# jltsiren/gcsa2

Measured on AMD Instinct MI355X. Metric: kmer_find_queries_per_sec, higher is better.
Workload: dtype u64; 1 GPU; whole-human-pangenome-sized index: order-17 de Bruijn graph of a degree-34 LFSR cycle of 5726623061 positions + junction edges between existing nodes (80 per mille of the candidates): 5726623061 path nodes, 6184749492 edges = 1.080 n; one batch of 100000000 x 32-mer find() sharded over 1 GPU(s), pattern set S (walks through the graph); edges=6184749492, queries_total=100000000, queries_per_gpu=100000000, pattern_len=32, index_bytes_hbm=209905278128, pair_block_bytes=61083979776, single_block_bytes=13362120576, kmer_table_k=16, block_bytes=128, pattern_set=S

## Files before the change

gcsa2_amd/csrc/gcsa2_hip.hip:

```cpp
#include "layout.hpp"
#include "sdsl_reader.hpp"
#include "sdsl_writer.hpp"
#include "../../include/gcsa2_hip.h"

#include <hipcub/hipcub.hpp>
#include <chrono>
#include <condition_variable>
#include <cstdio>
#include <cstdlib>
#include <cstring>
#include <algorithm>
#include <functional>
#include <atomic>
#include <memory>
#include <mutex>
#include <new>
#include <random>
#include <string>
#include <thread>
#include <unordered_set>
#include <vector>

using namespace g2;

// ... 2 lines not shown
#include "kernels_extend.hpp"
#include "kernels_locate.hpp"
#include "kernels_locate_max.hpp"
#include "kernels_mem.hpp"
#include "kernels_windows.hpp"
#include "kernels_lcp.hpp"
#include "kernels_submem.hpp"
#include "kernels_seeds.hpp"
#include "kernels_support.hpp"
#include "kernels_classes.hpp"
#include "kernels_mailbox.hpp"
#include "kernels_build.hpp"


constexpr unsigned RESULT_SLOTS = 1024;

struct Staging
{
  hipStream_t stream = nullptr;
  char* d = nullptr; size_t d_cap = 0;
  char* h = nullptr; size_t h_cap = 0;
  char* z = nullptr;
};

struct gcsa2_index
{
  int device = 0;
  DevImage img;
  void* d_base = nullptr;
  void* d_kmer = nullptr;
  void* d_pred4 = nullptr;
  void* d_locate = nullptr;
  void* d_jump = nullptr;
  void* d_pairs = nullptr;
  hipMemPool_t pool = nullptr;
  unsigned long long* d_slots = nullptr;
  unsigned long long* h_slots = nullptr;
  mutable std::atomic<unsigned> next_slot{0};
  mutable std::atomic<unsigned long long> next_ticket{1};
  mutable std::atomic<int> single_backoff{0};
  struct Mailbox { MailSlot* slot = nullptr; hipStream_t stream = nullptr; std::mutex lock; unsigned long long ticket = 0, launches = 0, calls = 0; bool failed = false; };
  mutable Mailbox mail;
  mutable std::mutex staging_lock;
  mutable std::vector<Staging*> staging_pool;
  int compute_units = 256;
  u64 bytes = 0;
  u64 order = 0;
  struct PipeSet { char* h = nullptr; char* d = nullptr; hipEvent_t done = nullptr; bool busy = false; u64 first = 0, count = 0; };
  struct PipeLane { hipStream_t stream = nullptr; PipeSet set[2]; };
  mutable std::mutex pipe_lock;
  mutable std::vector<PipeLane> pipe;
  struct Arena { char* base = nullptr; size_t bytes = 0; };
  mutable std::mutex arena_lock;
  mutable std::vector<Arena> arenas;
  struct Tuning
  {
    u32 cool_down = COOL_DOWN;
    u32 ms_refill_at = MS_REFILL_AT;
    u64 ms_grid = 0;
    u64 locate_split = (u64(1) << 31) - 1;
    u64 locate_split_queries = u64(1) << 30;
    u64 pipe_chunk = u64(1) << 18;
    u32 pipe_lanes = 6;
    u32 ms_threads = 4;
    u64 kmer_piece = u64(1) << 27;
    u64 ms_piece_bytes = u64(32) << 20;
    bool pipe_blocking = false;
    bool ms_pieces = true;
    bool zero_copy = true;
    u32 seed_wide = (u32(1) << 24) - 1;
    bool locate_trace = false;
    u32 split_target = SPLIT_TARGET;
    u32 split_skew = BIG_SEGMENT;
    bool locate_fused_compact = true;
    bool locate_single = true;
    bool locate_fuse = true;
    u64 fuse_above = BIG_SEGMENT;
    bool mailbox = true;
    u64 mailbox_park_us = 200;
    u64 mailbox_life_ms = 20;
    bool locate_in_place = true;
    size_t arena_cap = size_t(24) << 30;
    u64 budget_bytes = 0;
  } tune;
};

struct gcsa2_locate_job
{
  int device = 0;
  u64 nq = 0, total = 0;
  u64* d_offsets = nullptr;
  u64* d_values = nullptr;
  hipStream_t stream = nullptr;
};

namespace {

thread_local std::string g_error;

int fail(int code, const std::string& msg) { g_error = msg; return code; }

#define HIP_TRY(expr) do { hipError_t e_ = (expr); if(e_ != hipSuccess) { \
  return fail(e_ == hipErrorOutOfMemory ? GCSA2_ERR_OUT_OF_MEMORY : GCSA2_ERR_HIP, \
              std::string(#expr) + ": " + hipGetErrorString(e_)); } } while(0)

inline unsigned grid_for(u64 n) { return unsigned((n + TPB - 1) / TPB); }

inline u64 budget_left(const gcsa2_index* ix) { return ix->tune.budget_bytes > ix->bytes ? ix->tune.budget_bytes - ix->bytes : 0; }

constexpr bool JUMP_DEFAULT_FIND_ONLY = true;
inline bool jump_table_fits(u64 bytes, u64 free_bytes, u64 total_bytes) { return bytes <= free_bytes && free_bytes - bytes >= total_bytes / 16; }

inline void launch_walk(const gcsa2_index* ix, const u64* d_ranges, u64 nq, const u64* node_off, const u64* raw_off,
                        u64 total_nodes, u64* values, u64* owners, hipStream_t stream);


inline u64 pair_block_bytes_of(const DevImage& img) { return 16 * (img.n / PAIR_BITS + 1) * FLB_BYTES; }
inline bool pair_blocks_possible(const DevImage& img) { return img.sigma >= 5 && img.n > 0 && 16 * (img.n / PAIR_BITS + 1) < u64(PAIR_FLAG); }
inline bool seed_table_possible(const DevImage& img) { return img.sigma >= 5 && (img.n > img.e ? img.n : img.e) + 2 < (u64(1) << SEED_SP_BITS); }
inline bool locate_table_possible(const DevImage& img) { return img.has_samples && img.pred4 != nullptr && img.n > 0; }

void drop_pair_blocks(gcsa2_index* ix)
{
  if(ix->d_pairs != nullptr) { (void)hipFree(ix->d_pairs); ix->d_pairs = nullptr; ix->bytes -= pair_block_bytes_of(ix->img); }
  ix->img.flp = nullptr; ix->img.flp_nblocks = 0;
}

hipError_t make_pair_blocks(gcsa2_index* ix)
{
  drop_pair_blocks(ix);
  DevImage& img = ix->img;
  const u64 nb = img.n / PAIR_BITS + 1, pair_bytes = pair_block_bytes_of(img);
  hipError_t e = hipMalloc(&ix->d_pairs, pair_bytes);
  if(e == hipSuccess)
  {
    img.flp_nblocks = nb;
    const u64 slice = u64(1) << 20;
    for(u64 first = 0; first < nb && e == hipSuccess; first += slice)
    {
      const u64 count = (nb - first < slice ? nb - first : slice);
      hipLaunchKernelGGL(k_build_pair_blocks, dim3(unsigned(count), 4), dim3(unsigned(PAIR_BITS)), 0, nullptr, img, first, static_cast<u64*>(ix->d_pairs));
      e = hipGetLastError();
    }
    if(e == hipSuccess) { e = hipDeviceSynchronize(); }
  }
  if(e != hipSuccess)
  {
    if(ix->d_pairs != nullptr) { (void)hipFree(ix->d_pairs); ix->d_pairs = nullptr; }
    img.flp_nblocks = 0; (void)hipGetLastError();
    return e;
  }
  img.flp = static_cast<const u64*>(ix->d_pairs);
  ix->bytes += pair_bytes;
  return hipSuccess;
}

void drop_seed_table(gcsa2_index* ix)
{
  if(ix->d_kmer != nullptr) { (void)hipFree(ix->d_kmer); ix->d_kmer = nullptr; ix->bytes -= u64(8) << (2 * ix->img.kmer_k); }
  ix->img.kmer_table = nullptr; ix->img.kmer_k = 0;
}

hipError_t make_seed_table(gcsa2_index* ix, u32 k)
{
  drop_seed_table(ix);
  DevImage& img = ix->img;
// ... 475 lines not shown
  {
    if(v->char2comp[b] >= v->sigma) { return fail(GCSA2_ERR_INVALID_ARGUMENT, "alpha.char2comp maps a byte to a comp >= sigma"); }
  }
  for(u64 c = 0; c < v->sigma; c++)
  {
    if(v->C[c] > v->C[c + 1]) { return fail(GCSA2_ERR_INVALID_ARGUMENT, "alpha.C is not non-decreasing"); }
  }
  if(v->C[v->sigma] != v->edges) { return fail(GCSA2_ERR_INVALID_ARGUMENT, "alpha.C[sigma] differs from header.edges"); }
  if(v->sampled_path_bits != nullptr)
  {
    if(v->stored_samples == nullptr || v->sample_bits == nullptr || v->sample_width == 0 || v->sample_width > 64)
    {
      return fail(GCSA2_ERR_INVALID_ARGUMENT, "samples: missing array or sample width out of range");
    }
  }
  if(v->extra_filter_bits != nullptr && (v->extra_values_bits == nullptr || v->redundant_bits == nullptr))
  {
    return fail(GCSA2_ERR_INVALID_ARGUMENT, "counters: missing array");
  }
  if(v->lcp_data != nullptr)
  {
    if(v->lcp_offsets == nullptr || v->lcp_levels == 0) { return fail(GCSA2_ERR_INVALID_ARGUMENT, "LCP: missing offsets"); }
    if(v->lcp_branching < 2) { return fail(GCSA2_ERR_INVALID_ARGUMENT, "LCP: branching factor below 2"); }
    if(v->path_nodes > 0 && v->lcp_size != v->path_nodes) { return fail(GCSA2_ERR_INVALID_ARGUMENT, "LCP: header.size differs from the number of path nodes (an .lcp file of another index?)"); }
    u64 level_size = v->lcp_size, at = 0, top_size = 0;
    for(u64 l = 0; l < v->lcp_levels; l++)
    {
      if(v->lcp_offsets[l] != at) { return fail(GCSA2_ERR_INVALID_ARGUMENT, "LCP: offsets do not match the level sizes implied by the branching factor"); }
      at += level_size; top_size = level_size;
      if(l + 1 < v->lcp_levels && level_size <= 1) { return fail(GCSA2_ERR_INVALID_ARGUMENT, "LCP: levels above the root"); }
      level_size = (level_size + v->lcp_branching - 1) / v->lcp_branching;
    }
    if(v->lcp_offsets[v->lcp_levels] != at) { return fail(GCSA2_ERR_INVALID_ARGUMENT, "LCP: offsets do not match the level sizes implied by the branching factor"); }
    if(top_size > 1) { return fail(GCSA2_ERR_INVALID_ARGUMENT, "LCP: the top level is not a single root"); }
  }
  int count = gcsa2_device_count();
  if(count <= 0) { return fail(GCSA2_ERR_NO_DEVICE, "no HIP device visible: " + g_error); }
  if(device < 0 || device >= count) { return fail(GCSA2_ERR_INVALID_ARGUMENT, "device index out of range"); }

  if(v->sigma * (v->path_nodes / FLB_BITS + 1) >= u64(PAIR_FLAG) || v->lcp_size / 16 + 16 >= u64(PAIR_FLAG))
  {
    return fail(GCSA2_ERR_INVALID_ARGUMENT, "index too large: the block and LCP-window indices of the fetch keep two flag bits");
  }
  if(v->path_nodes > MAX_PATH_NODES || v->edges > 2 * MAX_PATH_NODES)
  {
    return fail(GCSA2_ERR_INVALID_ARGUMENT, "index of more than 2^38 path nodes: beyond what one device holds and what the block indices of this build address");
  }
  gcsa2_index* ix = new(std::nothrow) gcsa2_index();
  if(ix == nullptr) { return fail(GCSA2_ERR_OUT_OF_MEMORY, "host allocation failed"); }
  ix->device = device; ix->order = v->order;
  {
    auto knob = [](const char* name, long fallback, long lo, long hi) -> long
    {
      const char* e = std::getenv(name);
      long val = (e != nullptr && *e != 0 ? std::atol(e) : fallback);
      return val < lo ? lo : (val > hi ? hi : val);
    };
    ix->tune.cool_down = u32(knob("GCSA2_COOL_DOWN", COOL_DOWN, 0, 1000));
    ix->tune.ms_refill_at = u32(knob("GCSA2_MS_REFILL_AT", MS_REFILL_AT, 1, 64));
    ix->tune.ms_grid = u64(knob("GCSA2_MS_GRID", 0, 0, long(1) << 30));
    ix->tune.locate_split = u64(knob("GCSA2_LOCATE_SPLIT", (long(1) << 31) - 1, 2, (long(1) << 31) - 1));
    ix->tune.locate_split_queries = u64(knob("GCSA2_LOCATE_SPLIT_QUERIES", long(1) << 30, 1, long(1) << 30));
    ix->tune.zero_copy = (knob("GCSA2_ZERO_COPY", 1, 0, 1) != 0);
    ix->tune.pipe_lanes = u32(knob("GCSA2_PIPE_LANES", 6, 1, 16));
    ix->tune.pipe_chunk = u64(1) << knob("GCSA2_PIPE_CHUNK", 18, 15, 20);
    ix->tune.pipe_blocking = (knob("GCSA2_PIPE_BLOCKING", 0, 0, 1) != 0);
    ix->tune.ms_pieces = (knob("GCSA2_MS_PIECES", 1, 0, 1) != 0);
    ix->tune.ms_piece_bytes = u64(knob("GCSA2_MS_PIECE_MB", 32, 1, 1024)) << 20;
    ix->tune.ms_threads = u32(knob("GCSA2_MS_THREADS", 4, 1, 16));
    ix->tune.kmer_piece = u64(knob("GCSA2_KMER_PIECE", long(1) << 27, 4, long(1) << 27));
    ix->tune.locate_trace = (knob("GCSA2_LOCATE_TRACE", 0, 0, 1) != 0);
    ix->tune.locate_single = (knob("GCSA2_LOCATE_SINGLE", 1, 0, 1) != 0);
    ix->tune.locate_fused_compact = (knob("GCSA2_LOCATE_FUSED_COMPACT", 1, 0, 1) != 0);
    ix->tune.locate_fuse = (knob("GCSA2_LOCATE_FUSE", 1, 0, 1) != 0);
    ix->tune.fuse_above = u64(knob("GCSA2_LOCATE_FUSE_ABOVE", BIG_SEGMENT, 1, long(1) << 40));
    ix->tune.locate_in_place = (knob("GCSA2_LOCATE_IN_PLACE", 1, 0, 1) != 0);
    ix->tune.mailbox = (knob("GCSA2_MAILBOX", 1, 0, 1) != 0);
    ix->tune.mailbox_park_us = u64(knob("GCSA2_MAILBOX_PARK_US", 200, 1, 1000000));
    ix->tune.mailbox_life_ms = u64(knob("GCSA2_MAILBOX_LIFE_MS", 20, 1, 10000));
    ix->tune.split_skew = u32(knob("GCSA2_SPLIT_SKEW", BIG_SEGMENT, 16, BIG_SEGMENT));
    ix->tune.split_target = u32(knob("GCSA2_SPLIT_TARGET", SPLIT_TARGET, 1, 4096));
    ix->tune.arena_cap = size_t(knob("GCSA2_ARENA_CAP_MB", 24576, 0, long(1) << 20)) << 20;
    ix->tune.seed_wide = u32(knob("GCSA2_SEED_WIDE", long(SEED_WIDE), 2, long(SEED_WIDE)));
    {
      const char* b = std::getenv("GCSA2_MEMORY_BUDGET_MB");
      const double mb = (b != nullptr && *b != 0 ? std::atof(b) : 0.0);
      ix->tune.budget_bytes = (mb > 0.0 ? u64(mb * 1048576.0) : 0);
    }
  }
  std::memset(&ix->img, 0, sizeof(DevImage));
  DevImage& img = ix->img;
  img.n = v->path_nodes; img.e = v->edges; img.sigma = v->sigma; img.fast_chars = v->fast_chars;
  for(u64 c = 0; c <= v->sigma; c++) { img.C[c] = v->C[c]; }
  std::memcpy(img.char2comp, v->char2comp, 256);

  try
  {
    Planner pl;
    std::vector<BVPlan> bwt(v->sigma);
    for(u64 c = 0; c < v->sigma; c++)
    {
      bwt[c] = plan_bv(pl, img.n, false);
      if(c > 0 && bwt[c].blocks_off != bwt[0].blocks_off + c * (bwt[0].nblocks * BLOCK_WORDS))
      {
        delete ix; return fail(GCSA2_ERR_INVALID_ARGUMENT, "internal: B_c stride mismatch");
      }
    }
    BVPlan edges = plan_bv(pl, img.e, false);
    img.flb_nblocks = img.n / FLB_BITS + 1;
    const u64 flb_off = pl.reserve(v->sigma * img.flb_nblocks * FLB_WORDS, FLB_WORDS);
    BVPlan sampled, samples, xfilter, xvalues, redundant;
    u64 stored_off = 0, lcp_off = 0, stored_words = 0, max_bits = (img.n > img.e ? img.n : img.e);
    img.has_samples = (v->sampled_path_bits != nullptr);
    if(img.has_samples)
    {
      sampled = plan_bv(pl, img.n, false);
      samples = plan_bv(pl, v->sample_count, true);
      stored_words = (v->sample_count * v->sample_width + 63) / 64;
      stored_off = pl.reserve(stored_words + 2);
      img.sample_count = v->sample_count; img.sample_width = v->sample_width;
      if(v->sample_count > max_bits) { max_bits = v->sample_count; }
    }
    img.has_counters = (v->extra_filter_bits != nullptr);
    if(img.has_counters)
    {
      xfilter = plan_bv(pl, img.n, false);
      xvalues = plan_bv(pl, v->extra_values_len, true);
      redundant = plan_bv(pl, v->redundant_len, true);
      if(v->extra_values_len > max_bits) { max_bits = v->extra_values_len; }
      if(v->redundant_len > max_bits) { max_bits = v->redundant_len; }
    }
    img.has_lcp = (v->lcp_data != nullptr);
    if(img.has_lcp)
    {
      img.lcp_size = v->lcp_size; img.lcp_branching = v->lcp_branching; img.lcp_levels = v->lcp_levels;
      img.lcp_shift = 0;
      if((v->lcp_branching & (v->lcp_branching - 1)) == 0) { while((u64(1) << img.lcp_shift) < v->lcp_branching) { img.lcp_shift++; } }
      for(u64 l = 0; l <= v->lcp_levels; l++) { img.lcp_offsets[l] = v->lcp_offsets[l]; }
      img.lcp_values = v->lcp_offsets[v->lcp_levels];
      lcp_off = pl.reserve((img.lcp_values + 7) / 8 + 18);
    }

    DeviceGuard guard(device);
    if(!guard.ok) { delete ix; return fail(GCSA2_ERR_HIP, "hipSetDevice failed"); }
    {
      int cus = 0;
      if(hipDeviceGetAttribute(&cus, hipDeviceAttributeMultiprocessorCount, device) == hipSuccess && cus > 0) { ix->compute_units = cus; }
      hipMemPoolProps props;
      std::memset(&props, 0, sizeof(props));
      props.allocType = hipMemAllocationTypePinned;
      props.handleTypes = hipMemHandleTypeNone;
      props.location.type = hipMemLocationTypeDevice;
      props.location.id = device;
      if(hipMemPoolCreate(&ix->pool, &props) == hipSuccess && ix->pool != nullptr)
      {
        uint64_t keep = ~uint64_t(0);
        (void)hipMemPoolSetAttribute(ix->pool, hipMemPoolAttrReleaseThreshold, &keep);
      }
      else { ix->pool = nullptr; }
      (void)hipGetLastError();
    }
    ix->bytes = pl.words * sizeof(u64);
    hipError_t e = hipMalloc(&ix->d_base, ix->bytes > 0 ? ix->bytes : 8);
    if(e != hipSuccess) { delete ix; return fail(GCSA2_ERR_OUT_OF_MEMORY, std::string("hipMalloc(image): ") + hipGetErrorString(e)); }
    e = hipMemset(ix->d_base, 0, ix->bytes > 0 ? ix->bytes : 8);
    if(e == hipSuccess) { e = hipMalloc(reinterpret_cast<void**>(&ix->d_slots), RESULT_SLOTS * TOTAL_WORDS * sizeof(unsigned long long)); }
// ... 280 lines not shown
  HIP_TRY(hipDeviceSynchronize());
  release_host_staging(ix);
  if(ix->pool != nullptr) { HIP_TRY(hipMemPoolTrimTo(ix->pool, 0)); }
  return GCSA2_OK;
}

int gcsa2_index_set_pipeline(gcsa2_index* ix, int lanes, int chunk_log2, int blocking)
{
  if(ix == nullptr) { return fail(GCSA2_ERR_INVALID_ARGUMENT, "null index"); }
  if(lanes > 16 || chunk_log2 > 20 || (chunk_log2 > 0 && chunk_log2 < 15)) { return fail(GCSA2_ERR_INVALID_ARGUMENT, "host pipeline: lanes 1..16, chunk_log2 15..20"); }
  const int rc = gcsa2_index_trim(ix);
  if(rc != GCSA2_OK) { return rc; }
  std::lock_guard<std::mutex> hold(ix->pipe_lock);
  if(lanes > 0) { ix->tune.pipe_lanes = u32(lanes); }
  if(chunk_log2 > 0) { ix->tune.pipe_chunk = u64(1) << chunk_log2; }
  if(blocking >= 0) { ix->tune.pipe_blocking = (blocking != 0); }
  return GCSA2_OK;
}

void gcsa2_index_destroy(gcsa2_index* ix)
{
  if(ix == nullptr) { return; }
  DeviceGuard guard(ix->device);
  mailbox_stop(ix, true);
  if(ix->d_base) { (void)hipFree(ix->d_base); }
  if(ix->d_kmer) { (void)hipFree(ix->d_kmer); }
  if(ix->d_pred4) { (void)hipFree(ix->d_pred4); }
  if(ix->d_locate) { (void)hipFree(ix->d_locate); }
  if(ix->d_jump) { (void)hipFree(ix->d_jump); }
  if(ix->d_pairs) { (void)hipFree(ix->d_pairs); }
  if(ix->d_slots) { (void)hipFree(ix->d_slots); }
  if(ix->h_slots) { (void)hipHostFree(ix->h_slots); }
  if(ix->pool) { (void)hipDeviceSynchronize(); (void)hipMemPoolDestroy(ix->pool); }
  release_host_staging(ix);
  delete ix;
}

int gcsa2_mailbox_stats(const gcsa2_index* ix, uint64_t* calls, uint64_t* launches)
{
  if(ix == nullptr || calls == nullptr || launches == nullptr) { return fail(GCSA2_ERR_INVALID_ARGUMENT, "null argument"); }
  std::lock_guard<std::mutex> hold(ix->mail.lock);
  *calls = ix->mail.calls; *launches = ix->mail.launches;
  return GCSA2_OK;
}

uint64_t gcsa2_size(const gcsa2_index* ix) { return ix->img.n; }
uint64_t gcsa2_edge_count(const gcsa2_index* ix) { return ix->img.e; }
uint64_t gcsa2_order(const gcsa2_index* ix) { return ix->order; }
uint64_t gcsa2_sample_count(const gcsa2_index* ix) { return ix->img.sample_count; }
uint64_t gcsa2_sample_bits(const gcsa2_index* ix) { return ix->img.sample_width; }
int gcsa2_device(const gcsa2_index* ix) { return ix->device; }
uint64_t gcsa2_device_bytes(const gcsa2_index* ix) { return ix->bytes; }
uint64_t gcsa2_block_bits(const gcsa2_index*) { return BLOCK_BITS; }


#define CHECK_INDEX(ix) do { if((ix) == nullptr) { return fail(GCSA2_ERR_INVALID_ARGUMENT, "null index"); } } while(0)
#define LAUNCH_CHECK(name) do { hipError_t e_ = hipGetLastError(); if(e_ != hipSuccess) { \
  return fail(GCSA2_ERR_HIP, std::string(name) + ": " + hipGetErrorString(e_)); } } while(0)

}

namespace {

template<class Launch>
int simple_batch(const gcsa2_index* ix, const uint64_t* in, u64 in_words, uint64_t* out, u64 out_words, u64 nq, const char* name, Launch launch)
{
  DeviceGuard guard(ix->device);
  Lease lease(ix);
  HIP_TRY(lease.begin(Lease::need(in_words * nq * 8) + Lease::need(out_words * nq * 8), true));
  u64* d_in = lease.dev<u64>(in_words * nq); u64* d_out = lease.dev<u64>(out_words * nq);
  HIP_TRY(lease.up(d_in, in, in_words * nq * sizeof(u64)));
  launch(d_in, d_out, lease.stream());
  { hipError_t e_ = hipGetLastError(); if(e_ != hipSuccess) { return fail(GCSA2_ERR_HIP, std::string(name) + ": " + hipGetErrorString(e_)); } }
  HIP_TRY(lease.down(out, d_out, out_words * nq * sizeof(u64)));
  HIP_TRY(lease.finish());
  return GCSA2_OK;
}

template<bool STATS>
void launch_find2(const gcsa2_index* ix, unsigned grid, hipStream_t st, const uint8_t* d_patterns, const uint64_t* d_offsets, u64 nq,
                  uint64_t* d_ranges, unsigned long long* d_stats, const u32* perm)
{
  const bool jump = ix->img.jump_tab != nullptr, pair = ix->img.flp != nullptr;
#define G2_FIND2(J, P) hipLaunchKernelGGL((k_find2<STATS, J, P>), dim3(grid), dim3(TPB2), 0, st, \
                                          ix->img, d_patterns, d_offsets, nq, d_ranges, d_stats, perm)
  if(jump && pair) { G2_FIND2(true, true); }
  else if(jump) { G2_FIND2(true, false); }
  else if(pair) { G2_FIND2(false, true); }
  else { G2_FIND2(false, false); }
#undef G2_FIND2
}

}

extern "C" {

int gcsa2_find_device(const gcsa2_index* ix, const uint8_t* d_patterns, const uint64_t* d_offsets,
                      uint64_t nq, uint64_t* d_ranges, void* stream)
{
  CHECK_INDEX(ix);
  DeviceGuard guard(ix->device);
  if(nq == 0) { return GCSA2_OK; }
  launch_find2<false>(ix, unsigned((nq + TPB2 - 1) / TPB2), static_cast<hipStream_t>(stream), d_patterns, d_offsets, nq, d_ranges,
                      nullptr, nullptr);
  LAUNCH_CHECK("k_find2");
  return GCSA2_OK;
}

int gcsa2_find_packed_device(const gcsa2_index* ix, const uint64_t* d_codes, uint64_t pattern_length, uint64_t nq, uint64_t* d_ranges, void* stream)
{
  CHECK_INDEX(ix);
  DeviceGuard guard(ix->device);
  if(nq == 0) { return GCSA2_OK; }
  if(pattern_length == 0 || pattern_length >= (u64(1) << 32)) { return fail(GCSA2_ERR_INVALID_ARGUMENT, "packed patterns: the common length must be 1 .. 2^32 - 1"); }
  if(ix->img.sigma < 5) { return fail(GCSA2_ERR_INVALID_ARGUMENT, "packed patterns need the comps 1..4"); }
  const unsigned grid = unsigned((nq + TPB2 - 1) / TPB2);
  const u8* codes = reinterpret_cast<const u8*>(d_codes);
  const u64* length = reinterpret_cast<const u64*>(pattern_length);
  hipStream_t st = static_cast<hipStream_t>(stream);
  if(ix->img.flp != nullptr)
  {
    hipLaunchKernelGGL((k_find2<false, false, true, true>), dim3(grid), dim3(TPB2), 0, st, ix->img, codes, length, nq, d_ranges, (unsigned long long*)nullptr, (const u32*)nullptr);
  }
  else
  {
    hipLaunchKernelGGL((k_find2<false, false, false, true>), dim3(grid), dim3(TPB2), 0, st, ix->img, codes, length, nq, d_ranges, (unsigned long long*)nullptr, (const u32*)nullptr);
  }
  LAUNCH_CHECK("k_find2<packed>");
  return GCSA2_OK;
}

int gcsa2_find_device_variant(const gcsa2_index* ix, int variant, const uint8_t* d_patterns, const uint64_t* d_offsets,
                              uint64_t nq, uint64_t* d_ranges, void* stream)
{
  CHECK_INDEX(ix);
  if(nq == 0) { return GCSA2_OK; }
  if(variant == 2) { return gcsa2_find_device(ix, d_patterns, d_offsets, nq, d_ranges, stream); }
  if(variant == 4)
  {
    if(nq >= (u64(1) << 31)) { return fail(GCSA2_ERR_BUFFER_TOO_SMALL, "length-bucketed find is limited to 2^31 queries per launch"); }
    hipStream_t st = static_cast<hipStream_t>(stream);
    DeviceGuard guard(ix->device);
    u32 *len_in = nullptr, *len_out = nullptr, *idx_in = nullptr, *idx_out = nullptr;
    void* tmp = nullptr;
    size_t tmp_bytes = 0;
    HIP_TRY(hipcub::DeviceRadixSort::SortPairs(nullptr, tmp_bytes, len_in, len_out, idx_in, idx_out, int(nq), 0, 32, st));
    HIP_TRY(pool_alloc(ix, reinterpret_cast<void**>(&len_in), 4 * nq * sizeof(u32), st));
    HIP_TRY(pool_alloc(ix, &tmp, tmp_bytes, st));
    len_out = len_in + nq; idx_in = len_out + nq; idx_out = idx_in + nq;
    hipLaunchKernelGGL(k_pattern_lengths, dim3(grid_for(nq)), dim3(TPB), 0, st, d_offsets, nq, len_in, idx_in);
    hipError_t e = hipcub::DeviceRadixSort::SortPairs(tmp, tmp_bytes, len_in, len_out, idx_in, idx_out, int(nq), 0, 32, st);
    if(e == hipSuccess)
    {
      launch_find2<false>(ix, unsigned((nq + TPB2 - 1) / TPB2), st, d_patterns, d_offsets, nq, d_ranges, nullptr, idx_out);
      e = hipGetLastError();
    }
    (void)hipFreeAsync(tmp, st); (void)hipFreeAsync(len_in, st);
    if(e != hipSuccess) { return fail(GCSA2_ERR_HIP, std::string("length-bucketed find: ") + hipGetErrorString(e)); }
    return GCSA2_OK;
  }
  return fail(GCSA2_ERR_INVALID_ARGUMENT, "unknown find variant (2: default, 4: queries ordered by pattern length first)");
}

int gcsa2_find_stats_device(const gcsa2_index* ix, const uint8_t* d_patterns, const uint64_t* d_offsets,
                            uint64_t nq, uint64_t* d_ranges, uint64_t* d_stats, void* stream)
{
  CHECK_INDEX(ix);
  DeviceGuard guard(ix->device);
// ... 4794 lines not shown
```

gcsa2_amd/csrc/kernels_find.hpp:

```cpp
#pragma once

#include "kernels_common.hpp"

using namespace g2;

namespace {

constexpr u64 SEED_SP_BITS = 40, SEED_SP_MASK = (u64(1) << SEED_SP_BITS) - 1, SEED_WIDE = (u64(1) << 24) - 1;
__device__ __forceinline__ u64 seed_pack(u64 sp, u64 ep, u64 wide)
{
  const u64 len = ep + 1 - sp;
  return (sp & SEED_SP_MASK) | ((len < wide ? len : SEED_WIDE) << SEED_SP_BITS);
}

__global__ __launch_bounds__(TPB) void k_seed_level(DevImage img, u32 j, u64 first, u64 last, u64* __restrict__ table)
{
  const u64 tix = first + u64(blockIdx.x) * TPB + threadIdx.x;
  if(tix >= last) { return; }
  u64 sp, ep;
  if(j == 0) { const u32 c = 1 + u32(tix & 3); sp = img.crange[2 * c]; ep = img.crange[2 * c + 1]; }
  else
  {
    const u64 prev = table[tix & ((u64(1) << (2 * j)) - 1)];
    u32 from = j;
// ... 175 lines not shown
  __builtin_amdgcn_wave_barrier();
  const u32 lds_base = __builtin_amdgcn_readfirstlane(u32(reinterpret_cast<size_t>(wave_stage)));
  const u32 group = lane >> 3;
  const u64 chunk = u64(((lane & 7) ^ (group & 7)) * 16);
  u64 src[8];
#pragma unroll
  for(u32 j = 0; j < 8; j++) { src[j] = wave_addr[8 * j + group]; }
#pragma unroll
  for(u32 j = 0; j < 8; j++)
  {
    __builtin_amdgcn_global_load_lds((const __attribute__((address_space(1))) void*)(src[j] + chunk),
                                     (__attribute__((address_space(3))) void*)(size_t(lds_base + j * 1024u)), 16, 0, 0);
  }
}
__device__ __forceinline__ void fetch_blocks_wait()
{
  __builtin_amdgcn_s_waitcnt(0x0F70);
  __builtin_amdgcn_wave_barrier();
}
template<bool PAIR = false, bool LCPW = false>
__device__ __forceinline__ void fetch_blocks_direct(const u64* __restrict__ flb, u32 idx, bool need, ulonglong2* wave_stage, u32 lane,
                                                    const u64* __restrict__ flp, const u8* __restrict__ lcp, u64* wave_addr)
{
  fetch_blocks_issue<PAIR, LCPW>(flb, idx, need, wave_stage, lane, flp, lcp, wave_addr);
  fetch_blocks_wait();
}

__device__ __forceinline__ void read_block(const ulonglong2* wave_stage, u32 lane, ulonglong2 (&blk)[8])
{
#pragma unroll
  for(u32 k = 0; k < 8; k++) { blk[k] = wave_stage[lane * 8 + (k ^ (lane & 7))]; }
}

__device__ __forceinline__ u64 staged_word(const ulonglong2* wave_stage, u32 lane, u32 w)
{
  return reinterpret_cast<const u64*>(wave_stage)[(lane * 8 + ((w >> 1) ^ (lane & 7))) * 2 + (w & 1)];
}

__device__ __forceinline__ PairEnd eval_staged(const ulonglong2* wave_stage, u32 lane, bool pair, u32 r, bool ep_side)
{
  const ulonglong2 head = wave_stage[lane * 8 + (lane & 7)];
  const ulonglong2 tail = wave_stage[lane * 8 + (7 ^ (lane & 7))];
  const u32 wq = r >> 6, width = (pair ? 8u : 10u), mask = (pair ? 0xFFu : 0x3FFu);
  const u64 part = (u64(1) << (r & 63)) - 1;
  const u64 cum_rank = (pair ? tail.y : tail.x), cum_edges = (pair ? tail.y >> 40 : tail.y);
  const u64 bword = staged_word(wave_stage, lane, 2 + wq);
  const u32 ones = (wq == 0 ? 0u : u32(cum_rank >> (width * (wq - 1))) & mask) + u32(__popcll(bword & part));
  PairEnd out;
  out.raw = head.x + ones; out.bits = 0;
  u32 back = (ep_side ? 1u : 0u);
  if(pair)
  {
    const u64 dword = staged_word(wave_stage, lane, 5 + wq), qword = staged_word(wave_stage, lane, 8 + wq);
    const u32 qb = (wq == 0 ? 0u : u32(tail.y >> (16 + 8 * (wq - 1))) & 0xFF) + u32(__popcll(qword & part));
    const u32 qt = u32(tail.y >> 32) & 0xFF;
    const u32 dbit = (ep_side ? u32((dword >> (r & 63)) & 1) : 0u);
    out.bits = qb | ((qt - qb) << 8) | (dbit << 16);
    back = (ep_side ? 1u - dbit : 0u);
  }
  const u64 ncnt = head.y & ~PREV_BIT;
  if(back > ones) { out.node = ncnt - (head.y >> 63); return out; }
  const u32 k = ones - back, kq = k >> 6;
  const u64 kpart = (u64(1) << (k & 63)) - 1;
  const u64 eword = staged_word(wave_stage, lane, (pair ? 11u : 8u) + kq);
  out.node = ncnt + (kq == 0 ? 0u : u32(cum_edges >> (width * (kq - 1))) & mask) + u32(__popcll(eword & kpart));
  return out;
}

constexpr u32 JUMP_MAX = 8;
constexpr u64 JUMP_NODE_BITS = 36, JUMP_NODE_MASK = (u64(1) << JUMP_NODE_BITS) - 1;
__device__ __forceinline__ u64 jt_end(ulonglong2 e) { return e.x & JUMP_NODE_MASK; }
__device__ __forceinline__ u64 jt_after4(ulonglong2 e) { return (e.x >> 36) | ((e.y & 0xFF) << 28); }
__device__ __forceinline__ u64 jt_after2(ulonglong2 e) { return (e.y >> 8) & JUMP_NODE_MASK; }
__device__ __forceinline__ u32 jt_labels(ulonglong2 e) { return u32(e.y >> 44) & 0xFFFF; }
__device__ __forceinline__ u32 jt_len(ulonglong2 e) { return u32(e.y >> 60); }
__device__ __forceinline__ ulonglong2 jt_make(u64 end, u64 after4, u64 after2, u32 labels, u32 len)
{
  return make_ulonglong2(end | (after4 << 36), (after4 >> 28) | (after2 << 8) | (u64(labels) << 44) | (u64(len) << 60));
}

constexpr int FIND_WAVES = 4;
constexpr int JUMP_WAVES = 5;
template<bool STATS, bool JUMP = false, bool PAIR = false, bool PACKED = false>
__global__ __launch_bounds__(TPB2, JUMP ? JUMP_WAVES : (STATS ? 4 : FIND_WAVES)) void k_find2(DevImage img, const u8* __restrict__ patterns,
                                               const u64* __restrict__ offsets, u64 nq,
                                               u64* __restrict__ out, unsigned long long* __restrict__ stats,
                                               const u32* __restrict__ perm)
{
  constexpr bool WINDOW = true;
  __shared__ ulonglong2 stage[TPB2 * 8];
  __shared__ Tables2 t;
  if(threadIdx.x < 2 * MAX_SIGMA) { t.crange[threadIdx.x] = img.crange[threadIdx.x]; }
  t.c2c[threadIdx.x] = img.char2comp[threadIdx.x];
  t.c2c[threadIdx.x + TPB2] = img.char2comp[threadIdx.x + TPB2];
  __syncthreads();

  const u32 lane = threadIdx.x & 63;
  ulonglong2* wave_stage = stage + (threadIdx.x & ~63u) * 8;
  [[maybe_unused]] u64* wave_addr = nullptr;
  if constexpr(JUMP)
  {
    __shared__ u64 addr_table[TPB2];
    wave_addr = addr_table + (threadIdx.x & ~63u);
  }
  u64 blocks = 0, steps = 0, lookups = 0, jumps = 0;
  [[maybe_unused]] u64 fetch_steps = 0, second_fetches = 0, wide_seeds = 0;
  [[maybe_unused]] unsigned int* touched = nullptr;
  if constexpr(STATS) { touched = reinterpret_cast<unsigned int*>(stats[7]); }

  u64 q = ~u64(0), sp = 0, ep = img.n - 1, i = 0;
  const u8* p = patterns;
  bool done = true;
  [[maybe_unused]] bool tried = false;
  [[maybe_unused]] bool no_jump = false;
  [[maybe_unused]] u64 win_code = 0;
  [[maybe_unused]] u32 win_used = ~u32(0), win_bad = 0;
  [[maybe_unused]] u32 force_single = 0;
  u64 word = 0, word_addr = ~u64(0);
  auto byte_at = [&](u64 pos) -> u32
  {
    u64 addr = reinterpret_cast<u64>(p) + pos, aligned = addr & ~u64(7);
    if(aligned != word_addr) { word = *reinterpret_cast<const u64*>(aligned); word_addr = aligned; }
    return u32(word >> ((addr & 7) * 8)) & 0xFF;
  };
  auto start = [&](u64 query)
  {
    q = query; sp = 0; ep = img.n - 1; i = 0; done = true; word_addr = ~u64(0); tried = false; no_jump = false; win_used = ~u32(0);
    force_single = 0;
    u64 begin = 0, len = 0;
    if constexpr(PACKED)
    {
      len = reinterpret_cast<u64>(offsets);
      begin = q * ((len + 31) >> 5) * 8;
    }
    else { begin = offsets[q]; len = offsets[q + 1] - begin; }
    if(len > 0 && img.n > 0)
    {
      p = patterns + begin;
      const u32 k = img.kmer_k;
      bool seeded = false;
      if(k > 0 && len >= k)
      {
        u64 tix = 0;
        bool fast = true;
        if constexpr(PACKED) { tix = *reinterpret_cast<const u64*>(p) & ((u64(1) << (2 * k)) - 1); }
        else
        {
          for(u32 j = 0; j < k; j++)
          {
            u32 comp = t.c2c[byte_at(len - 1 - j)];
            fast = fast && (comp - 1 < 4);
            tix |= u64((comp - 1) & 3) << (2 * j);
          }
        }
        if(fast)
        {
          const u64 entry = img.kmer_table[tix];
          sp = entry & SEED_SP_MASK; ep = sp + (entry >> SEED_SP_BITS) - 1;
          fast = (entry >> SEED_SP_BITS) != SEED_WIDE;
          if(STATS) { lookups++; wide_seeds += (fast ? 0 : 1); }
        }
        if(fast)
        {
          i = len - k; seeded = true;
        }
      }
      if(!seeded)
      {
        i = len - 1;
        u32 comp = 0;
        if constexpr(PACKED) { comp = 1 + u32(*reinterpret_cast<const u64*>(p) & 3); }
        else { comp = t.c2c[byte_at(i)]; }
        sp = t.crange[2 * comp]; ep = t.crange[2 * comp + 1];
      }
      done = range_empty(sp, ep) || i == 0;
    }
  };

  {
    const u64 gid = u64(blockIdx.x) * TPB2 + threadIdx.x;
    if(gid < nq) { start(perm != nullptr ? u64(perm[gid]) : gid); }
  }

  while(true)
  {
    if(!__any(!done)) { break; }
    bool jumping = false;
    ulonglong2 entry = make_ulonglong2(0, 0);
    if constexpr(JUMP)
    {
      jumping = !done && sp == ep && i >= 2 && !tried && !no_jump;
      entry = img.jump_tab[jumping ? sp : 0];
    }
    if constexpr(WINDOW)
    {
      if constexpr(PACKED)
      {
        if(!done && win_used > 24)
        {
          const u64 total = reinterpret_cast<u64>(offsets), words = (total + 31) >> 5;
          const u64 t0 = total - i, w = t0 >> 5;
          const u32 s = u32(t0 & 31);
          const u64* code = reinterpret_cast<const u64*>(p);
          const u64 c0 = code[w], c1 = (w + 1 < words ? code[w + 1] : 0);
          win_code = (s == 0 ? c0 : (c0 >> (2 * s)) | (c1 << (64 - 2 * s)));
          win_bad = 0; win_used = 0;
        }
      }
      else if(!done && win_used > 24)
      {
        win_used = 0; win_code = 0; win_bad = 0;
        const u64 count = (i < 32 ? i : 32), low = reinterpret_cast<u64>(p) + i - count, base = low & ~u64(7);
        u64 w[5];
        const u64 last = (low + count - 1) & ~u64(7);
#pragma unroll
        for(u32 k = 0; k < 5; k++) { const u64 a = base + 8 * k; w[k] = *reinterpret_cast<const u64*>(a < last ? a : last); }
        for(u32 r = 0; r < count; r++)
        {
          const u64 at = (low - base) + (count - 1 - r);
          u64 word = w[0];
#pragma unroll
          for(u32 k = 1; k < 5; k++) { if((at >> 3) == k) { word = w[k]; } }
          const u32 c = u32(t.c2c[u32(word >> ((at & 7) * 8)) & 0xFF]) - 1;
          win_code |= u64(c & 3) << (2 * r);
          win_bad |= u32(c < 4 ? 0 : 1) << r;
        }
      }
    }
    const bool stepping = !done && !jumping;
    u32 comp = 0, r_sp = 0, r_ep = 0, idx_sp = 0, idx_ep = 0;
    bool pair = false;
    if(stepping)
    {
      if constexpr(PAIR)
      {
        if(force_single == 0 && i >= 2)
        {
          const u32 r = win_used;
          pair = ((win_bad >> r) & 3) == 0;
          if(pair)
          {
            const u32 c2 = u32(win_code >> (2 * r)) & 3, c1 = u32(win_code >> (2 * r + 2)) & 3;
            u32 b_sp, b_ep;
            pair_block_of(sp, b_sp, r_sp); pair_block_of(ep + 1, b_ep, r_ep);
            const u32 first = (c1 * 4 + c2) * u32(img.flp_nblocks);
            idx_sp = (first + b_sp) | PAIR_FLAG; idx_ep = (first + b_ep) | PAIR_FLAG;
          }
        }
      }
      if(!pair)
      {
        i--;
        if constexpr(PAIR) { force_single -= (force_single > 0 ? 1 : 0); }
        if constexpr(WINDOW)
        {
          const u32 r = win_used++;
          if((win_bad >> r) & 1)
          {
            const u64 addr = reinterpret_cast<u64>(p) + i;
            comp = t.c2c[u32(*reinterpret_cast<const u64*>(addr & ~u64(7)) >> ((addr & 7) * 8)) & 0xFF];
          }
          else { comp = 1 + (u32(win_code >> (2 * r)) & 3); }
        }
        else { comp = t.c2c[byte_at(i)]; }
        u32 b_sp, b_ep;
        flb_block_of(sp, b_sp, r_sp); flb_block_of(ep + 1, b_ep, r_ep);
        idx_sp = comp * u32(img.flb_nblocks) + b_sp; idx_ep = comp * u32(img.flb_nblocks) + b_ep;
      }
    }
    PairEnd p_sp = {0, 0, 0}, p_ep = {0, 0, 0};
    const bool need2 = stepping && idx_ep != idx_sp;
    if(STATS && stepping)
    {
      blocks += 1 + (need2 ? 1 : 0); fetch_steps++; second_fetches += (need2 ? 1 : 0);
      if(touched != nullptr)
      {
        const u32 singles = u32(img.sigma) * u32(img.flb_nblocks);
        const u32 a = (idx_sp & PAIR_FLAG) ? singles + (idx_sp & ~PAIR_FLAG) : idx_sp;
        atomicOr(touched + (a >> 5), 1u << (a & 31));
        if(need2) { const u32 b = (idx_ep & PAIR_FLAG) ? singles + (idx_ep & ~PAIR_FLAG) : idx_ep; atomicOr(touched + (b >> 5), 1u << (b & 31)); }
      }
    }
    if constexpr(JUMP)
    {
      fetch_blocks_direct<PAIR>(img.flb, idx_sp, stepping, wave_stage, lane, img.flp, nullptr, wave_addr);
      if(stepping)
      {
        p_sp = eval_staged(wave_stage, lane, PAIR && pair, r_sp, false);
        if(idx_ep == idx_sp) { p_ep = eval_staged(wave_stage, lane, PAIR && pair, r_ep, true); }
      }
      if(__any(need2))
      {
        fetch_blocks_direct<PAIR>(img.flb, idx_ep, need2, wave_stage, lane, img.flp, nullptr, wave_addr);
        if(need2) { p_ep = eval_staged(wave_stage, lane, PAIR && pair, r_ep, true); }
      }
    }
    else
    {
      ulonglong2 blk[8];
      fetch_blocks<PAIR>(img.flb, idx_sp, stepping, wave_stage, lane, img.flp);
      if(stepping)
      {
        read_block(wave_stage, lane, blk);
        if(PAIR && pair)
        {
          p_sp = eval_pair(blk, r_sp, false);
          if(idx_ep == idx_sp) { p_ep = eval_pair(blk, r_ep, true); }
        }
        else
        {
          eval_endpoint(blk, r_sp, 0, p_sp.raw, p_sp.node);
          if(idx_ep == idx_sp) { eval_endpoint(blk, r_ep, 1, p_ep.raw, p_ep.node); }
        }
      }
      if(__any(need2))
      {
        __builtin_amdgcn_wave_barrier();
        fetch_blocks<PAIR>(img.flb, idx_ep, need2, wave_stage, lane, img.flp);
        if(need2)
        {
          read_block(wave_stage, lane, blk);
          if(PAIR && pair) { p_ep = eval_pair(blk, r_ep, true); }
          else { eval_endpoint(blk, r_ep, 1, p_ep.raw, p_ep.node); }
        }
      }
    }
    __builtin_amdgcn_wave_barrier();
    if(stepping)
    {
      if(PAIR && pair)
      {
        u64 a = 0, b = 0;
        const u32 outcome = pair_outcome(p_sp, p_ep, idx_ep == idx_sp, a, b);
        if(outcome == 2)
        {
          sp = p_sp.node; ep = p_ep.node; i -= 2; win_used += 2; done = (i == 0);
          if(STATS) { steps += 2; }
          if constexpr(JUMP) { tried = false; }
        }
        else if(outcome == 1)
        {
          sp = a; ep = b; i -= 2; win_used += 2; done = true;
          if(STATS) { steps += 2; }
        }
        else { force_single = 2; }
      }
      else
      {
        if(STATS) { steps++; }
        u64 a = p_sp.raw, b = p_ep.raw - 1;
        if(range_empty(a, b)) { sp = a; ep = b; done = true; }
        else { sp = p_sp.node; ep = p_ep.node; done = (i == 0); }
        if constexpr(JUMP) { tried = false; }
      }
    }
    if constexpr(JUMP)
    {
      if(jumping)
      {
        const u32 len = jt_len(entry), r = win_used;
        u32 bad8 = (win_bad >> r) & 0xFF;
        bad8 = (bad8 | (bad8 << 4)) & 0x0F0F; bad8 = (bad8 | (bad8 << 2)) & 0x3333; bad8 = (bad8 | (bad8 << 1)) & 0x5555;
        const u32 diff = (u32(win_code >> (2 * r)) ^ jt_labels(entry)) & 0xFFFF;
        const u32 bad = ((diff | (diff >> 1)) & 0x5555) | bad8;
        u32 usable = (bad != 0 ? u32(__ffs(int(bad)) - 1) >> 1 : 8u);
        usable = (usable < len ? usable : len);
        usable = (usable < i ? usable : u32(i));
        u32 take = (usable == len ? len : (usable >= 4 ? 4u : (usable >= 2 ? 2u : 0u)));
        if(STATS) { jumps++; }
        if(take > 0)
        {
          sp = ep = (take == len ? jt_end(entry) : (take == 4 ? jt_after4(entry) : jt_after2(entry)));
          i -= take; win_used += take; done = (i == 0);
          tried = (take == len && len < JUMP_MAX);
          if(STATS) { steps += take; }
        }
        else
        {
          tried = true;
          no_jump = (len > 0);
        }
      }
    }
  }
  {
    const u64 gid = u64(blockIdx.x) * TPB2 + threadIdx.x;
    if(gid < nq) { reinterpret_cast<ulonglong2*>(out)[perm != nullptr ? u64(perm[gid]) : gid] = make_ulonglong2(sp, ep); }
  }
  if(STATS)
  {
    for(int o = 32; o > 0; o >>= 1)
    {
      blocks += __shfl_down(blocks, o, 64); steps += __shfl_down(steps, o, 64); lookups += __shfl_down(lookups, o, 64);
      jumps += __shfl_down(jumps, o, 64); fetch_steps += __shfl_down(fetch_steps, o, 64);
      second_fetches += __shfl_down(second_fetches, o, 64); wide_seeds += __shfl_down(wide_seeds, o, 64);
    }
    if(lane == 0)
    {
      atomicAdd(stats, (unsigned long long)blocks); atomicAdd(stats + 1, (unsigned long long)steps);
      atomicAdd(stats + 2, (unsigned long long)lookups); atomicAdd(stats + 3, (unsigned long long)jumps);
      atomicAdd(stats + 4, (unsigned long long)fetch_steps); atomicAdd(stats + 5, (unsigned long long)second_fetches);
      atomicAdd(stats + 6, (unsigned long long)wide_seeds);
    }
  }
}

__global__ __launch_bounds__(192) void k_build_pair_blocks(DevImage img, u64 first, u64* __restrict__ out)
{
  __shared__ u64 s_ecnt[4], s_p[4][3], s_q[3], s_e[4][4];
  const u64 b = first + blockIdx.x, nb = img.flp_nblocks;
  const u32 c2 = 1 + blockIdx.y, r = threadIdx.x;
  const u64 i = b * PAIR_BITS + r, n = img.n, e = img.e;
  const bool valid = i <= n;
  u64 rk = 0;
  const bool q = bv_get_rank(bwt_of(img, c2), valid ? (i < n ? i : n) : 0, rk) && i < n;
  const u64 x = img.C[c2] + rk;
  u64 u = 0;
  const bool ebit = bv_get_rank(img.edges, clampu(x, e), u) && x < e;
  const bool split = (x >= 1 && x - 1 < e) && !bv_get(img.edges, x - 1);
  const u64 qw = __ballot(valid && q);
#pragma unroll
  for(u32 c1 = 1; c1 <= 4; c1++)
  {
    u64 rc = 0;
    const bool bc = bv_get_rank(bwt_of(img, c1), clampu(u, n), rc) && u < n;
    const u64 pw = __ballot(valid && q && ebit && bc), dw = __ballot(valid && split && bc);
    u64* dst = out + (u64((c1 - 1) * 4 + (c2 - 1)) * nb + b) * FLB_WORDS;
    if((r & 63) == 0) { dst[2 + (r >> 6)] = pw; dst[5 + (r >> 6)] = dw; dst[8 + (r >> 6)] = qw; s_p[c1 - 1][r >> 6] = pw; s_q[r >> 6] = qw; }
    if(r == 0)
    {
      const u64 ecnt = img.C[c1] + rc;
      u64 ncnt = 0;
      (void)bv_get_rank(img.edges, clampu(ecnt, e), ncnt);
      const u64 prev = (ecnt >= 1 && ecnt - 1 < e && bv_get(img.edges, ecnt - 1)) ? PREV_BIT : 0;
      dst[0] = ecnt; dst[1] = ncnt | prev;
      s_ecnt[c1 - 1] = ecnt;
    }
  }
  __syncthreads();
  if(r < 16)
  {
    const u32 c1 = 1 + r / 4, k = r % 4;
    u64* dst = out + (u64((c1 - 1) * 4 + (c2 - 1)) * nb + b) * FLB_WORDS;
    const u64 slice = bv_bits64(img.edges, s_ecnt[c1 - 1] + 64 * k);
    dst[11 + k] = slice; s_e[c1 - 1][k] = slice;
  }
  __syncthreads();
  if(r < 4)
  {
    u64* dst = out + (u64(r * 4 + (c2 - 1)) * nb + b) * FLB_WORDS;
    const u64 p0 = __popcll(s_p[r][0]), p1 = p0 + __popcll(s_p[r][1]);
    const u64 q0 = __popcll(s_q[0]), q1 = q0 + __popcll(s_q[1]), q2 = q1 + __popcll(s_q[2]);
    const u64 e0 = __popcll(s_e[r][0]), e1 = e0 + __popcll(s_e[r][1]), e2 = e1 + __popcll(s_e[r][2]);
    dst[15] = p0 | (p1 << 8) | (q0 << 16) | (q1 << 24) | (q2 << 32) | (e0 << 40) | (e1 << 48) | (e2 << 56);
  }
}

__global__ __launch_bounds__(TPB) void k_pattern_lengths(const u64* __restrict__ offsets, u64 nq,
                                                         u32* __restrict__ len, u32* __restrict__ idx)
{
  u64 q = u64(blockIdx.x) * TPB + threadIdx.x;
  if(q >= nq) { return; }
  u64 l = offsets[q + 1] - offsets[q];
  len[q] = u32(l > 0xFFFFFFFFull ? 0xFFFFFFFFull : l);
  idx[q] = u32(q);
}

// ... 185 lines not shown
```

gcsa2_amd/csrc/layout.hpp:

```cpp
#pragma once

#include <hip/hip_runtime.h>
#include <stdint.h>

namespace g2 {

typedef uint64_t u64;
typedef uint32_t u32;
typedef uint8_t  u8;

constexpr u64 BLOCK_WORDS   = 8;
constexpr u64 PAYLOAD_WORDS = 7;
constexpr u64 BLOCK_BITS    = 448;
constexpr u64 BLOCK_BYTES   = 64;
constexpr u64 SELECT_SAMPLE = 448;
constexpr u64 FLB_WORDS     = 16;
constexpr u64 FLB_BITS      = 384;
constexpr u64 FLB_PAYLOAD   = 6;
constexpr u64 FLB_BYTES     = 128;
constexpr u64 PREV_BIT      = u64(1) << 63;
constexpr u64 PAIR_BITS     = 192;
constexpr u32 PAIR_WORDS    = 3;
constexpr u32 PAIR_FLAG     = u32(1) << 30;
constexpr u32 LCP_FLAG      = u32(1) << 31;
constexpr int MAX_SIGMA     = 16;
constexpr int MAX_LCP_LEVELS = 64;

struct DevBV
{
  const u64* blocks;
  const u32* hints;
  u64 size, nblocks, ones;
};

struct DevImage
{
  u64 n, e, sigma, fast_chars;
  u64 C[MAX_SIGMA + 1];
  DevBV bwt[MAX_SIGMA];
  DevBV edges;
  const u64* flb;
  u64 flb_nblocks;
  const u64* flp;
  u64 flp_nblocks;
  u64 crange[2 * MAX_SIGMA];
  const u64* pred4;
  const u64* kmer_table;
  u32 kmer_k;
  u32 seed_wide;
  u32 lcp_shift;
  const ulonglong2* jump_tab;
  const u64* locate_tab;
  DevBV sampled;
  DevBV samples;
  const u64* stored;
  u64 sample_count, sample_width;
  DevBV xfilter;
  DevBV xvalues;
  DevBV redundant;
  const u8* lcp;
  u64 lcp_size, lcp_branching, lcp_levels, lcp_values;
  u64 lcp_offsets[MAX_LCP_LEVELS + 1];
  int has_samples, has_counters, has_lcp;
  u8 char2comp[256];
};


struct Block { u64 w[8]; };

__device__ __forceinline__ Block load_block(const u64* p)
{
  const ulonglong2* q = reinterpret_cast<const ulonglong2*>(p);
  ulonglong2 a = q[0], b = q[1], c = q[2], d = q[3];
  Block r;
  r.w[0] = a.x; r.w[1] = a.y; r.w[2] = b.x; r.w[3] = b.y;
  r.w[4] = c.x; r.w[5] = c.y; r.w[6] = d.x; r.w[7] = d.y;
  return r;
}

__device__ __forceinline__ u64 rank_in_block(const Block& b, u32 r)
{
  u64 res = b.w[0];
  u32 wq = r >> 6, rb = r & 63;
  u64 part = (u64(1) << rb) - 1;
#pragma unroll
  for(u32 j = 0; j < 7; j++)
  {
    u64 m = (j < wq ? ~u64(0) : (j == wq ? part : u64(0)));
    res += __popcll(b.w[j + 1] & m);
  }
  return res;
}

__device__ __forceinline__ u64 block_of(u64 i) { return i / BLOCK_BITS; }

__device__ __forceinline__ u64 bv_rank(const DevBV& bv, u64 i)
{
  u64 blk = block_of(i);
  Block b = load_block(bv.blocks + blk * BLOCK_WORDS);
  return rank_in_block(b, u32(i - blk * BLOCK_BITS));
}

__device__ __forceinline__ void bv_rank2(const DevBV& bv, u64 i, u64 j, u64& ri, u64& rj)
{
  u64 bi = block_of(i), bj = block_of(j);
  Block a = load_block(bv.blocks + bi * BLOCK_WORDS);
  ri = rank_in_block(a, u32(i - bi * BLOCK_BITS));
  if(bj == bi) { rj = rank_in_block(a, u32(j - bj * BLOCK_BITS)); }
  else
  {
    Block b = load_block(bv.blocks + bj * BLOCK_WORDS);
    rj = rank_in_block(b, u32(j - bj * BLOCK_BITS));
  }
}

__device__ __forceinline__ bool bv_get(const DevBV& bv, u64 i)
{
  u64 blk = block_of(i);
  u32 r = u32(i - blk * BLOCK_BITS);
  return (bv.blocks[blk * BLOCK_WORDS + 1 + (r >> 6)] >> (r & 63)) & 1;
}

__device__ __forceinline__ bool bv_get_rank(const DevBV& bv, u64 i, u64& rank)
{
  u64 blk = block_of(i);
  u32 r = u32(i - blk * BLOCK_BITS);
  Block b = load_block(bv.blocks + blk * BLOCK_WORDS);
  rank = rank_in_block(b, r);
  return (b.w[1 + (r >> 6)] >> (r & 63)) & 1;
}

__device__ __forceinline__ u32 select_in_word(u64 w, u32 k)
{
// ... 59 lines not shown
```

Baseline: 7.029 billion queries/s.

## Run multiple query generations per wave with prefetch of next query during jump search

For the jump-table find kernel, each wave now processes a sequence of query generations (64 queries each) instead of one query per thread, and while the current generation's block fetches are in flight it prefetches the next query's offsets, pattern words and k-mer seed entry. Results are written when a generation finishes. This aims to hide the latency of starting a new query behind the memory-bound search loop. It adds register pressure, splits fetch into issue/wait, and defaults to one generation, so the grid size is unchanged by default.

After: 6.887 billion queries/s. 2.0% lower.

```diff
diff --git a/gcsa2_amd/csrc/gcsa2_hip.hip b/gcsa2_amd/csrc/gcsa2_hip.hip
--- a/gcsa2_amd/csrc/gcsa2_hip.hip
+++ b/gcsa2_amd/csrc/gcsa2_hip.hip
@@ -108,6 +108,7 @@
     bool locate_in_place = true;
     size_t arena_cap = size_t(24) << 30;
     u64 budget_bytes = 0;
+    u32 find_gens = 0;
   } tune;
 };
 
@@ -749,6 +750,7 @@
     ix->tune.split_target = u32(knob("GCSA2_SPLIT_TARGET", SPLIT_TARGET, 1, 4096));
     ix->tune.arena_cap = size_t(knob("GCSA2_ARENA_CAP_MB", 24576, 0, long(1) << 20)) << 20;
     ix->tune.seed_wide = u32(knob("GCSA2_SEED_WIDE", long(SEED_WIDE), 2, long(SEED_WIDE)));
+    ix->tune.find_gens = u32(knob("GCSA2_FIND_GENERATIONS", 0, 0, 16));
     {
       const char* b = std::getenv("GCSA2_MEMORY_BUDGET_MB");
       const double mb = (b != nullptr && *b != 0 ? std::atof(b) : 0.0);
@@ -1195,8 +1197,15 @@
                   uint64_t* d_ranges, unsigned long long* d_stats, const u32* perm)
 {
   const bool jump = ix->img.jump_tab != nullptr, pair = ix->img.flp != nullptr;
+  DevImage img = ix->img;
+  if(jump)
+  {
+    const u32 gens = (ix->tune.find_gens > 0 ? ix->tune.find_gens : 1);
+    img.find_gens = gens;
+    grid = unsigned((nq + u64(TPB2) * gens - 1) / (u64(TPB2) * gens));
+  }
 #define G2_FIND2(J, P) hipLaunchKernelGGL((k_find2<STATS, J, P>), dim3(grid), dim3(TPB2), 0, st, \
-                                          ix->img, d_patterns, d_offsets, nq, d_ranges, d_stats, perm)
+                                          img, d_patterns, d_offsets, nq, d_ranges, d_stats, perm)
   if(jump && pair) { G2_FIND2(true, true); }
   else if(jump) { G2_FIND2(true, false); }
   else if(pair) { G2_FIND2(false, true); }
diff --git a/gcsa2_amd/csrc/kernels_find.hpp b/gcsa2_amd/csrc/kernels_find.hpp
--- a/gcsa2_amd/csrc/kernels_find.hpp
+++ b/gcsa2_amd/csrc/kernels_find.hpp
@@ -281,7 +281,7 @@
 constexpr int FIND_WAVES = 4;
 constexpr int JUMP_WAVES = 5;
 template<bool STATS, bool JUMP = false, bool PAIR = false, bool PACKED = false>
-__global__ __launch_bounds__(TPB2, JUMP ? JUMP_WAVES : (STATS ? 4 : FIND_WAVES)) void k_find2(DevImage img, const u8* __restrict__ patterns,
+__global__ __launch_bounds__(TPB2, JUMP && !STATS ? JUMP_WAVES : (STATS ? 4 : FIND_WAVES)) void k_find2(DevImage img, const u8* __restrict__ patterns,
                                                const u64* __restrict__ offsets, u64 nq,
                                                u64* __restrict__ out, unsigned long long* __restrict__ stats,
                                                const u32* __restrict__ perm)
@@ -376,6 +376,102 @@
     }
   };
 
+  [[maybe_unused]] u64 ord = 0;
+  [[maybe_unused]] u32 gens_left = 0;
+  [[maybe_unused]] u32 pf_stage = 2;
+  [[maybe_unused]] bool started = false;
+  [[maybe_unused]] u64 n_p = 0, n_len = 0, n_entry = 0, n_code = 0;
+  [[maybe_unused]] u32 n_bad = 0, n_info = 0;
+  [[maybe_unused]] auto next_live = [&]() -> bool { return ord + 64 < nq && n_len > 0 && img.n > 0; };
+  [[maybe_unused]] auto next_offsets = [&]()
+  {
+    if(ord + 64 < nq)
+    {
+      const u64 query = (perm != nullptr ? u64(perm[ord + 64]) : ord + 64);
+      n_p = offsets[query]; n_len = offsets[query + 1];
+    }
+  };
+  [[maybe_unused]] auto next_words = [&](u64 (&w)[5])
+  {
+    n_len -= n_p; n_p += reinterpret_cast<u64>(patterns);
+    if(next_live())
+    {
+      const u64 count = (n_len < 33 ? n_len : 33), low = n_p + n_len - count, base = low & ~u64(7);
+      const u64 last = (low + count - 1) & ~u64(7);
+#pragma unroll
+      for(u32 k = 0; k < 5; k++) { const u64 a = base + 8 * k; w[k] = *(const __attribute__((address_space(1))) u64*)(a < last ? a : last); }
+    }
+  };
+  [[maybe_unused]] auto next_build = [&](const u64 (&w)[5])
+  {
+    if(next_live())
+    {
+      const u32 count = u32(n_len < 33 ? n_len : 33), shift = u32((n_p + n_len - count) & 7);
+      u64 code = 0;
+      u32 bad = 0, far = 0, last = 0;
+#pragma unroll
+      for(u32 j = 0; j < 5; j++)
+      {
+        u64 word = w[j];
+#pragma unroll 1
+        for(u32 b = 0; b < 8; b++, word >>= 8)
+        {
+          const u32 d = count - 1 + shift - (8 * j + b);
+          if(d < count)
+          {
+            const u32 comp = t.c2c[u32(word) & 0xFF], c = comp - 1;
+            if(d == 0) { last = comp; }
+            if(d < 32) { code |= u64(c & 3) << (2 * d); bad |= u32(c < 4 ? 0 : 1) << d; } else { far = (c & 3) | (c < 4 ? 0 : 4); }
+          }
+        }
+      }
+      const u32 k = img.kmer_k;
+      const bool fast = k > 0 && n_len >= k && (bad & ((u32(1) << k) - 1)) == 0;
+      const u32 s = (fast ? k : 1), lead = (n_len > 33 ? s - 1 : 0);
+      n_code = ((code >> (2 * s)) | (u64(far & 3) << (64 - 2 * s))) << (2 * lead);
+      n_bad = ((bad >> s) | ((far >> 2) << (32 - s))) << lead;
+      n_info = lead | (last << 8) | (fast ? 1u << 16 : 0u);
+      if(fast) { n_entry = img.kmer_table[code & ((u64(1) << (2 * k)) - 1)]; }
+    }
+  };
+  [[maybe_unused]] auto next_begin = [&]()
+  {
+    sp = 0; ep = img.n - 1; i = 0; done = true;
+    tried = false; no_jump = false; force_single = 0;
+    if(next_live())
+    {
+      p = reinterpret_cast<const u8*>(n_p);
+      win_code = n_code; win_bad = n_bad; win_used = n_info & 0xFF;
+      const bool n_fast = (n_info >> 16) != 0;
+      bool seeded = false;
+      if(n_fast)
+      {
+        sp = n_entry & SEED_SP_MASK; ep = sp + (n_entry >> SEED_SP_BITS) - 1;
+        seeded = (n_entry >> SEED_SP_BITS) != SEED_WIDE;
+        if(STATS) { lookups++; wide_seeds += (seeded ? 0 : 1); }
+      }
+      if(seeded) { i = n_len - img.kmer_k; }
+      else
+      {
+        const u32 comp = (n_info >> 8) & 0xFF;
+        i = n_len - 1;
+        sp = t.crange[2 * comp]; ep = t.crange[2 * comp + 1];
+        if(n_fast) { win_used = ~u32(0); }
+      }
+      done = range_empty(sp, ep) || i == 0;
+    }
+  };
+
+  if constexpr(JUMP)
+  {
+    static_assert(!PACKED, "the JUMP form reads byte patterns");
+    const u32 gens = (img.find_gens > 0 ? img.find_gens : 1);
+    const u64 wave = __builtin_amdgcn_readfirstlane(u32(threadIdx.x >> 6)) + u64(blockIdx.x) * (TPB2 / 64);
+    const u64 first = wave * gens * 64;
+    ord = first + lane - 64;
+    if(first < nq) { gens_left = gens; pf_stage = 0; }
+  }
+  else
   {
     const u64 gid = u64(blockIdx.x) * TPB2 + threadIdx.x;
     if(gid < nq) { start(perm != nullptr ? u64(perm[gid]) : gid); }
@@ -383,7 +479,22 @@
 
   while(true)
   {
-    if(!__any(!done)) { break; }
+    if constexpr(JUMP)
+    {
+      if(!__any(!done))
+      {
+        if(started && ord < nq) { reinterpret_cast<ulonglong2*>(out)[perm != nullptr ? u64(perm[ord]) : ord] = make_ulonglong2(sp, ep); }
+        if(gens_left == 0) { break; }
+        if(pf_stage < 1) { next_offsets(); }
+        if(pf_stage < 2) { u64 w[5] = {0, 0, 0, 0, 0}; next_words(w); next_build(w); }
+        next_begin();
+        ord += 64; started = true;
+        gens_left = (__any(ord + 64 < nq) ? gens_left - 1 : 0);
+        pf_stage = (gens_left > 0 ? 0 : 2);
+        continue;
+      }
+    }
+    else if(!__any(!done)) { break; }
     bool jumping = false;
     ulonglong2 entry = make_ulonglong2(0, 0);
     if constexpr(JUMP)
@@ -482,7 +593,12 @@
     }
     if constexpr(JUMP)
     {
-      fetch_blocks_direct<PAIR>(img.flb, idx_sp, stepping, wave_stage, lane, img.flp, nullptr, wave_addr);
+      u64 next_w[5] = {0, 0, 0, 0, 0};
+      if(pf_stage == 1) { next_words(next_w); }
+      fetch_blocks_issue<PAIR>(img.flb, idx_sp, stepping, wave_stage, lane, img.flp, nullptr, wave_addr);
+      if(pf_stage == 0) { next_offsets(); pf_stage = 1; }
+      else if(pf_stage == 1) { next_build(next_w); pf_stage = 2; }
+      fetch_blocks_wait();
       if(stepping)
       {
         p_sp = eval_staged(wave_stage, lane, PAIR && pair, r_sp, false);
@@ -582,6 +698,7 @@
       }
     }
   }
+  if constexpr(!JUMP)
   {
     const u64 gid = u64(blockIdx.x) * TPB2 + threadIdx.x;
     if(gid < nq) { reinterpret_cast<ulonglong2*>(out)[perm != nullptr ? u64(perm[gid]) : gid] = make_ulonglong2(sp, ep); }
diff --git a/gcsa2_amd/csrc/layout.hpp b/gcsa2_amd/csrc/layout.hpp
--- a/gcsa2_amd/csrc/layout.hpp
+++ b/gcsa2_amd/csrc/layout.hpp
@@ -49,6 +49,7 @@
   u32 kmer_k;
   u32 seed_wide;
   u32 lcp_shift;
+  u32 find_gens;
   const ulonglong2* jump_tab;
   const u64* locate_tab;
   DevBV sampled;
```
